# david-zwicker/video-analysis

Hardware: AMD Instinct MI355X
Metric: frames/sec (bg-sub+blur+thresh+CCL) 1080p uint8 (higher is better)
Workload: dtype u8; 1 GPU; cfg3_1080p_full_chain: 1920x1080 uint8, batch 256/GPU, running-mean bg-sub (f64 state) + sigma=5 Gaussian (q8.8) + threshold 20 + 5x5 dilate/erode + 4-connected labelling + object counts; inputs resident in HBM; engine=bg=1 gauss=mfma-i8(ksize=31) thresh=20 morph=2 ccl=4, video=one clip per rank, overlap=off, world_size=1, backend=single process

## Files before the change

### video-analysis_amd/csrc/va_point.hip

```cpp
#include <math.h>

#include "va_common.h"

namespace va {

namespace {

constexpr int kBlock = 256;
constexpr int kVec = 8;

__device__ __forceinline__ uint8_t sat_u8_trunc(double d)
{
    const int v = (int)d;
    return (uint8_t)(v > 255 ? 255 : v);
}

template <int V>
__global__ void __launch_bounds__(kBlock)
bg_mean_u8_kernel(const uint8_t *__restrict__ frames, uint8_t *__restrict__ diff,
                  double *__restrict__ mean, long long n_seen, int n, size_t px)
{
    size_t i0 = ((size_t)blockIdx.x * kBlock + threadIdx.x) * V;
    if (i0 >= px)
        return;
    double m[V];
#pragma unroll
    for (int k = 0; k < V; k++)
        m[k] = mean[i0 + k];
    for (int f = 0; f < n; f++) {
        uint8_t p[V];
        if (V == 8) {
            uint2 v = *reinterpret_cast<const uint2 *>(frames + (size_t)f * px + i0);
            memcpy(p, &v, 8);
        } else {
            p[0] = frames[(size_t)f * px + i0];
        }
        const double dn = (double)(n_seen + f), dn1 = (double)(n_seen + f + 1);
        uint8_t o[V];
#pragma unroll
        for (int k = 0; k < V; k++) {
            double fr = (double)p[k];
            o[k] = sat_u8_trunc(fabs(fr - m[k]));
            m[k] = m[k] * dn / dn1 + fr / dn1;
        }
        if (diff) {
            if (V == 8) {
                uint2 v;
                memcpy(&v, o, 8);
                *reinterpret_cast<uint2 *>(diff + (size_t)f * px + i0) = v;
            } else {
                diff[(size_t)f * px + i0] = o[0];
            }
        }
    }
#pragma unroll
    for (int k = 0; k < V; k++)
        mean[i0 + k] = m[k];
}

__device__ __forceinline__ double div_by_uniform(double x, double d, double y)
{
    const double q = x * y;
    const double r = fma(-q, d, x);
    return fma(r, y, q);
}

__global__ void __launch_bounds__(kBlock)
bg_reciprocals_kernel(double *__restrict__ y, long long n_seen, int n)
{
    const int f = blockIdx.x * kBlock + threadIdx.x;
    if (f < n)
        y[f] = 1.0 / (double)(n_seen + f + 1);
}

struct RecipArgs {
    double r[256];
    double lo[256];
    __device__ double operator[](int f) const { return r[f]; }
};
__device__ __forceinline__ double clear_low9(double y)
{
    return __builtin_bit_cast(double, __builtin_bit_cast(unsigned long long, y) & ~0x1FFull);
}

__device__ __forceinline__ unsigned byte_lane(unsigned w, int k)
{
    return k == 3 ? w >> 24 : (w >> (8 * k)) & 0xFFu;
}
__device__ __forceinline__ unsigned pack_bytes(const int *d)
{
    const unsigned lo = __builtin_amdgcn_perm((unsigned)d[1], (unsigned)d[0], 0x0C0C0400u);
    const unsigned hi = __builtin_amdgcn_perm((unsigned)d[3], (unsigned)d[2], 0x0C0C0400u);
    return __builtin_amdgcn_perm(hi, lo, 0x05040100u);
}

constexpr int kAhead = 8;

template <int V> struct BgGroup {
    typedef unsigned int vec __attribute__((ext_vector_type(V / 4)));
    vec v[kAhead];
    template <bool CLAMP>
    __device__ __forceinline__ void load(const uint8_t *frames, size_t i0, size_t px, int f0, int n)
    {
#pragma unroll
        for (int j = 0; j < kAhead; j++)
            v[j] = __builtin_nontemporal_load(reinterpret_cast<const vec *>(
                frames + (size_t)(CLAMP ? min(f0 + j, n - 1) : f0 + j) * px + i0));
    }
};

template <int V, typename RECIP, bool BOUNDED, bool SPLIT, bool DIFF, bool FULL>
__device__ __forceinline__ void bg_mean_group(const BgGroup<V> &g, double (&m)[V], double &dn, const RECIP &recip,
                                              int f0, int cnt, uint8_t *diff, size_t i0, size_t px)
{
#pragma unroll
    for (int j = 0; j < kAhead; j++) {
        if (!FULL && j >= cnt)
            break;
        const int f = f0 + j;
        const double dn1 = dn + 1.0;
        const double y = recip[f];
        double yh = 0.0, yl = 0.0;
        if constexpr (SPLIT) {
            yh = clear_low9(y);
            yl = recip.lo[f];
        }
        typename BgGroup<V>::vec out;
#pragma unroll
        for (int w = 0; w < V / 4; w++) {
            int d[4];
#pragma unroll
            for (int b = 0; b < 4; b++) {
                const int k = 4 * w + b;
                const double fr = (double)byte_lane(g.v[j][w], b);
                if constexpr (DIFF) {
                    const int a = (int)fabs(fr - m[k]);
                    d[b] = BOUNDED ? a : min(a, 255);
                }
                double q2;
                if constexpr (SPLIT)
                    q2 = fma(fr, yl, fr * yh);
                else
                    q2 = div_by_uniform(fr, dn1, y);
                m[k] = div_by_uniform(m[k] * dn, dn1, y) + q2;
            }
            if constexpr (DIFF)
                out[w] = pack_bytes(d);
        }
        if constexpr (DIFF)
            __builtin_nontemporal_store(out, reinterpret_cast<typename BgGroup<V>::vec *>(diff + (size_t)f * px + i0));
        dn = dn1;
    }
}

template <int V, typename RECIP, bool BOUNDED, bool SPLIT, bool DIFF>
__global__ void __launch_bounds__(kBlock)
bg_mean_u8_fast_kernel(const uint8_t *__restrict__ frames, uint8_t *__restrict__ diff,
                       double *__restrict__ mean, const RECIP recip, double dn0, int n, size_t px)
{
    const size_t i0 = ((size_t)blockIdx.x * kBlock + threadIdx.x) * V;
    if (i0 >= px)
        return;
    double m[V];
#pragma unroll
    for (int k = 0; k < V; k++)
        m[k] = mean[i0 + k];
    double dn = dn0;
    BgGroup<V> a, b;
    a.template load<true>(frames, i0, px, 0, n);
    int f0 = 0;
    for (; f0 + 3 * kAhead <= n; f0 += 2 * kAhead) {
        b.template load<false>(frames, i0, px, f0 + kAhead, n);
        bg_mean_group<V, RECIP, BOUNDED, SPLIT, DIFF, true>(a, m, dn, recip, f0, kAhead, diff, i0, px);
        a.template load<false>(frames, i0, px, f0 + 2 * kAhead, n);
        bg_mean_group<V, RECIP, BOUNDED, SPLIT, DIFF, true>(b, m, dn, recip, f0 + kAhead, kAhead, diff, i0, px);
    }
    for (; f0 < n; f0 += kAhead) {
        const bool more = f0 + kAhead < n;
        if (more)
            b.template load<true>(frames, i0, px, f0 + kAhead, n);
        bg_mean_group<V, RECIP, BOUNDED, SPLIT, DIFF, false>(a, m, dn, recip, f0, min(kAhead, n - f0), diff, i0, px);
        if (more)
            a = b;
    }
#pragma unroll
    for (int k = 0; k < V; k++)
        mean[i0 + k] = m[k];
}

template <int V>
__global__ void __launch_bounds__(kBlock)
bg_static_u8_kernel(const uint8_t *__restrict__ frames, uint8_t *__restrict__ diff,
                    const double *__restrict__ bg, int n, size_t px)
{
    size_t i0 = ((size_t)blockIdx.x * kBlock + threadIdx.x) * V;
    if (i0 >= px)
        return;
    double m[V];
#pragma unroll
    for (int k = 0; k < V; k++)
        m[k] = bg[i0 + k];
    for (int f = 0; f < n; f++) {
        uint8_t p[V], o[V];
        if (V == 8) {
            uint2 v = *reinterpret_cast<const uint2 *>(frames + (size_t)f * px + i0);
            memcpy(p, &v, 8);
        } else {
            p[0] = frames[(size_t)f * px + i0];
        }
#pragma unroll
        for (int k = 0; k < V; k++)
            o[k] = sat_u8_trunc(fabs((double)p[k] - m[k]));
        if (V == 8) {
            uint2 v;
            memcpy(&v, o, 8);
            *reinterpret_cast<uint2 *>(diff + (size_t)f * px + i0) = v;
        } else {
            diff[(size_t)f * px + i0] = o[0];
        }
    }
}

template <int V>
__global__ void __launch_bounds__(kBlock)
bg_ema_u8_kernel(const uint8_t *__restrict__ frames, uint8_t *__restrict__ diff,
                 float *__restrict__ bg, long long n_seen, float rate, int n, size_t px)
{
    size_t i0 = ((size_t)blockIdx.x * kBlock + threadIdx.x) * V;
    if (i0 >= px)
        return;
    float m[V];
#pragma unroll
    for (int k = 0; k < V; k++)
        m[k] = bg[i0 + k];
    for (int f = 0; f < n; f++) {
        uint8_t p[V], o[V];
        if (V == 8) {
            uint2 v = *reinterpret_cast<const uint2 *>(frames + (size_t)f * px + i0);
            memcpy(p, &v, 8);
        } else {
            p[0] = frames[(size_t)f * px + i0];
        }
        const bool first = (n_seen + f) == 0;
#pragma unroll
        for (int k = 0; k < V; k++) {
            float fr = (float)p[k];
            if (first)
                m[k] = fr;
            float d = fr - m[k];
            float a = truncf(fabsf(d));
            o[k] = (uint8_t)(int)(a > 255.0f ? 255.0f : a);
            float step = rate * d;
            m[k] = m[k] + step;
        }
        if (diff) {
            if (V == 8) {
                uint2 v;
                memcpy(&v, o, 8);
                *reinterpret_cast<uint2 *>(diff + (size_t)f * px + i0) = v;
            } else {
                diff[(size_t)f * px + i0] = o[0];
            }
        }
    }
#pragma unroll
    for (int k = 0; k < V; k++)
        bg[i0 + k] = m[k];
}

template <int V>
__global__ void __launch_bounds__(kBlock)
bg_ema_f32_kernel(const float *__restrict__ frames, float *__restrict__ diff,
                  float *__restrict__ bg, long long n_seen, float rate, int n, size_t px)
{
    size_t i0 = ((size_t)blockIdx.x * kBlock + threadIdx.x) * V;
    if (i0 >= px)
        return;
    float m[V];
#pragma unroll
    for (int k = 0; k < V; k++)
        m[k] = bg[i0 + k];
    for (int f = 0; f < n; f++) {
        float p[V], o[V];
        if (V == 4) {
            float4 v = *reinterpret_cast<const float4 *>(frames + (size_t)f * px + i0);
            p[0] = v.x, p[1] = v.y, p[2] = v.z, p[3] = v.w;
        } else {
            p[0] = frames[(size_t)f * px + i0];
        }
        const bool first = (n_seen + f) == 0;
#pragma unroll
        for (int k = 0; k < V; k++) {
            if (first)
                m[k] = p[k];
            float d = p[k] - m[k];
            o[k] = fabsf(d);
            float step = rate * d;
            m[k] = m[k] + step;
        }
        if (diff) {
            if (V == 4)
                *reinterpret_cast<float4 *>(diff + (size_t)f * px + i0) =
                    make_float4(o[0], o[1], o[2], o[3]);
            else
                diff[(size_t)f * px + i0] = o[0];
        }
    }
#pragma unroll
    for (int k = 0; k < V; k++)
        bg[i0 + k] = m[k];
}

template <int V>
__global__ void __launch_bounds__(kBlock)
welford_u8_kernel(const uint8_t *__restrict__ frames, double *__restrict__ mean,
                  double *__restrict__ m2, long long n_seen, int n, size_t px)
{
    size_t i0 = ((size_t)blockIdx.x * kBlock + threadIdx.x) * V;
    if (i0 >= px)
        return;
    double m[V], q[V];
#pragma unroll
    for (int k = 0; k < V; k++) {
        m[k] = mean[i0 + k];
        q[k] = m2[i0 + k];
    }
    for (int f = 0; f < n; f++) {
        uint8_t p[V];
        if (V == 8) {
            uint2 v = *reinterpret_cast<const uint2 *>(frames + (size_t)f * px + i0);
            memcpy(p, &v, 8);
        } else {
            p[0] = frames[(size_t)f * px + i0];
        }
        const double dn1 = (double)(n_seen + f + 1);
#pragma unroll
        for (int k = 0; k < V; k++) {
            double fr = (double)p[k];
            double delta = fr - m[k];
            m[k] = m[k] + delta / dn1;
            q[k] = q[k] + delta * (fr - m[k]);
        }
    }
#pragma unroll
    for (int k = 0; k < V; k++) {
        mean[i0 + k] = m[k];
        m2[i0 + k] = q[k];
    }
}

template <class T>
__device__ __forceinline__ double quotient_as_numpy(T v, double dn1)
{
    return (double)v / dn1;
}
template <>
__device__ __forceinline__ double quotient_as_numpy<float>(float v, double dn1)
{
    return (double)(float)((double)v / (double)(float)dn1);
}

template <class T, bool WELFORD>
__global__ void __launch_bounds__(kBlock)
temporal_stats_kernel(const T *__restrict__ frames, double *__restrict__ mean, double *__restrict__ m2,
                      long long n_seen, int n, size_t px)
{
    const size_t i = (size_t)blockIdx.x * kBlock + threadIdx.x;
    if (i >= px)
        return;
    double m = mean[i], q = WELFORD ? m2[i] : 0.0;
    for (int f = 0; f < n; f++) {
        const T v = frames[(size_t)f * px + i];
        const double dn = (double)(n_seen + f), dn1 = (double)(n_seen + f + 1);
        if (WELFORD) {
            const double fr = (double)v, delta = fr - m;
            m = m + delta / dn1;
            q = q + delta * (fr - m);
        } else {
            m = m * dn / dn1 + quotient_as_numpy<T>(v, dn1);
        }
    }
    mean[i] = m;
    if (WELFORD)
        m2[i] = q;
}

__global__ void __launch_bounds__(kBlock)
threshold_u8_kernel(const uint8_t *__restrict__ src, uint8_t *__restrict__ dst, size_t count,
                    int thresh, int maxval, int vec_ok)
{
    size_t i0 = ((size_t)blockIdx.x * kBlock + threadIdx.x) * 16;
    if (i0 >= count)
        return;
    if (vec_ok && i0 + 16 <= count) {
        uint4 v = *reinterpret_cast<const uint4 *>(src + i0);
        uint8_t p[16];
        memcpy(p, &v, 16);
#pragma unroll
        for (int k = 0; k < 16; k++)
            p[k] = (int)p[k] > thresh ? (uint8_t)maxval : (uint8_t)0;
        memcpy(&v, p, 16);
        *reinterpret_cast<uint4 *>(dst + i0) = v;
    } else {
        for (size_t i = i0; i < count && i < i0 + 16; i++)
            dst[i] = (int)src[i] > thresh ? (uint8_t)maxval : (uint8_t)0;
    }
}

__global__ void __launch_bounds__(kBlock)
time_difference_kernel(const uint8_t *__restrict__ a, const uint8_t *__restrict__ b,
                       int16_t *__restrict__ out, size_t count, int vec_ok)
{
    size_t i0 = ((size_t)blockIdx.x * kBlock + threadIdx.x) * 8;
    if (i0 >= count)
        return;
    if (vec_ok && i0 + 8 <= count) {
        uint2 va_ = *reinterpret_cast<const uint2 *>(a + i0);
        uint2 vb_ = *reinterpret_cast<const uint2 *>(b + i0);
        uint8_t pa[8], pb[8];
        int16_t o[8];
        memcpy(pa, &va_, 8);
        memcpy(pb, &vb_, 8);
#pragma unroll
        for (int k = 0; k < 8; k++)
            o[k] = (int16_t)((int)pa[k] - (int)pb[k]);
        uint4 vo;
        memcpy(&vo, o, 16);
        *reinterpret_cast<uint4 *>(out + i0) = vo;
    } else {
        for (size_t i = i0; i < count && i < i0 + 8; i++)
            out[i] = (int16_t)((int)a[i] - (int)b[i]);
    }
}

__global__ void __launch_bounds__(kBlock)
mono_mean_kernel(const uint8_t *__restrict__ src, uint8_t *__restrict__ dst, size_t pixels)
{
    size_t i = (size_t)blockIdx.x * kBlock + threadIdx.x;
    if (i >= pixels)
        return;
    double s = (double)src[3 * i] + (double)src[3 * i + 1] + (double)src[3 * i + 2];
    dst[i] = (uint8_t)(int)(s / 3.0);
}

__global__ void __launch_bounds__(kBlock)
normalize_u8_kernel(const uint8_t *__restrict__ src, uint8_t *__restrict__ dst, size_t count,
                    double fmin, double fmax, double alpha, double tmin)
{
    size_t i = (size_t)blockIdx.x * kBlock + threadIdx.x;
    if (i >= count)
        return;
    double f = (double)src[i];
    f = f < fmin ? fmin : (f > fmax ? fmax : f);
    double v = (f - fmin) * alpha + tmin;
    int iv = (int)v;
    dst[i] = (uint8_t)iv;
}

}

template <int V, typename RECIP, bool BOUNDED, bool SPLIT>
static void launch_bg_fast(const uint8_t *fr, uint8_t *df, double *mean, const RECIP &recip, double dn0, int n,
                           size_t px, hipStream_t st)
{
    const int grid = cdiv((long long)(px / V), kBlock);
    if constexpr (BOUNDED)
        bg_mean_u8_fast_kernel<V, RECIP, true, SPLIT, true><<<grid, kBlock, 0, st>>>(fr, df, mean, recip, dn0, n, px);
    else if (df)
        bg_mean_u8_fast_kernel<V, RECIP, BOUNDED, SPLIT, true><<<grid, kBlock, 0, st>>>(fr, df, mean, recip, dn0, n, px);
    else
        bg_mean_u8_fast_kernel<V, RECIP, BOUNDED, SPLIT, false><<<grid, kBlock, 0, st>>>(fr, df, mean, recip, dn0, n, px);
}

size_t bg_scratch_bytes(int n) { return sizeof(double) * (size_t)(n > 0 ? n : 1); }

int launch_bg(int mode, int dtype, const void *frames, void *diff, void *state, int64_t n_seen,
              double rate, int n, size_t px, hipStream_t st, double *recip_scratch, bool mean_in_u8_range)
{
    VA_REQUIRE(frames && state, "va_bg_update: frames/state must not be NULL");
    VA_REQUIRE(n >= 0 && px > 0, "va_bg_update: bad sizes n=%d px=%zu", n, px);
    if (n == 0)
        return VA_OK;
    if (dtype == VA_U8) {
        const uint8_t *fr = (const uint8_t *)frames;
        uint8_t *df = (uint8_t *)diff;
        bool vec = (px % kVec == 0) && aligned(fr, 8) && (!df || aligned(df, 8));
        int grid = vec ? cdiv((long long)(px / kVec), kBlock) : cdiv((long long)px, kBlock);
        if (mode == VA_BG_MEAN) {
            const bool wide = px % 16 == 0 && aligned(fr, 16) && (!df || aligned(df, 16));
            const bool countable = n_seen >= -(1ll << 53) && n_seen <= (1ll << 53) - n;
            const bool bounded = mean_in_u8_range && df;
            const double dn0 = (double)n_seen;
            double *mean = (double *)state;
            if (vec && countable && n <= 256) {
                RecipArgs ra;
                for (int f = 0; f < 256; f++) {
                    const double d = (double)(n_seen + (f < n ? f : 0) + 1), y = 1.0 / d;
                    unsigned long long bits;
                    memcpy(&bits, &y, 8);
                    bits &= ~0x1FFull;
                    double yh;
                    memcpy(&yh, &bits, 8);
                    ra.r[f] = y;
                    ra.lo[f] = fma(y, fma(-d, y, 1.0), y - yh);
                }
#ifdef BG_NO_SPLIT
                const bool split = false;
#else
                const bool split = n_seen + n < (1ll << 40);
#endif
                if (wide && bounded && split)
                    launch_bg_fast<16, RecipArgs, true, true>(fr, df, mean, ra, dn0, n, px, st);
                else if (wide && bounded)
                    launch_bg_fast<16, RecipArgs, true, false>(fr, df, mean, ra, dn0, n, px, st);
                else if (wide && split)
                    launch_bg_fast<16, RecipArgs, false, true>(fr, df, mean, ra, dn0, n, px, st);
                else if (wide)
                    launch_bg_fast<16, RecipArgs, false, false>(fr, df, mean, ra, dn0, n, px, st);
                else
                    launch_bg_fast<8, RecipArgs, false, false>(fr, df, mean, ra, dn0, n, px, st);
            } else if (vec && countable && recip_scratch) {
                bg_reciprocals_kernel<<<cdiv(n, kBlock), kBlock, 0, st>>>(recip_scratch, n_seen, n);
                VA_LAUNCH_CHECK("bg_reciprocals_kernel");
                if (wide)
                    launch_bg_fast<16, const double *, false, false>(fr, df, mean, recip_scratch, dn0, n, px, st);
                else
                    launch_bg_fast<8, const double *, false, false>(fr, df, mean, recip_scratch, dn0, n, px, st);
            } else if (vec)
                bg_mean_u8_kernel<8><<<grid, kBlock, 0, st>>>(fr, df, (double *)state, n_seen, n, px);
            else
                bg_mean_u8_kernel<1><<<grid, kBlock, 0, st>>>(fr, df, (double *)state, n_seen, n, px);
        } else if (mode == VA_BG_EMA) {
            if (vec)
                bg_ema_u8_kernel<8><<<grid, kBlock, 0, st>>>(fr, df, (float *)state, n_seen,
                                                            (float)rate, n, px);
            else
                bg_ema_u8_kernel<1><<<grid, kBlock, 0, st>>>(fr, df, (float *)state, n_seen,
                                                            (float)rate, n, px);
        } else if (mode == VA_BG_STATIC) {
            VA_REQUIRE(df, "va_bg_update: static mode needs diff_out");
            if (vec)
                bg_static_u8_kernel<8><<<grid, kBlock, 0, st>>>(fr, df, (const double *)state, n, px);
            else
                bg_static_u8_kernel<1><<<grid, kBlock, 0, st>>>(fr, df, (const double *)state, n, px);
        } else {
            VA_REQUIRE(false, "va_bg_update: unsupported mode %d for u8 frames", mode);
        }
    } else if (dtype == VA_F32) {
        VA_REQUIRE(mode == VA_BG_EMA, "va_bg_update: float32 frames support VA_BG_EMA only");
        const float *fr = (const float *)frames;
        float *df = (float *)diff;
        bool vec = (px % 4 == 0) && aligned(fr, 16) && (!df || aligned(df, 16));
        int grid = vec ? cdiv((long long)(px / 4), kBlock) : cdiv((long long)px, kBlock);
        if (vec)
            bg_ema_f32_kernel<4><<<grid, kBlock, 0, st>>>(fr, df, (float *)state, n_seen,
                                                         (float)rate, n, px);
        else
            bg_ema_f32_kernel<1><<<grid, kBlock, 0, st>>>(fr, df, (float *)state, n_seen,
                                                         (float)rate, n, px);
    } else {
        VA_REQUIRE(false, "va_bg_update: unknown dtype %d", dtype);
    }
    VA_LAUNCH_CHECK("bg kernel");
    return VA_OK;
}

int launch_welford(const uint8_t *frames, double *mean, double *m2, int64_t n_seen, int n,
                   size_t px, hipStream_t st)
{
    VA_REQUIRE(frames && mean && m2, "va_welford_u8: NULL argument");
    if (n <= 0)
        return VA_OK;
    bool vec = (px % kVec == 0) && aligned(frames, 8);
    int grid = vec ? cdiv((long long)(px / kVec), kBlock) : cdiv((long long)px, kBlock);
    if (vec)
        welford_u8_kernel<8><<<grid, kBlock, 0, st>>>(frames, mean, m2, n_seen, n, px);
    else
        welford_u8_kernel<1><<<grid, kBlock, 0, st>>>(frames, mean, m2, n_seen, n, px);
    VA_LAUNCH_CHECK("welford_u8_kernel");
    return VA_OK;
}

int launch_temporal_stats(const void *frames, int dtype, double *mean, double *m2, int64_t n_seen, int n,
                          size_t px, hipStream_t st)
{
    VA_REQUIRE(frames && mean, "temporal statistics: NULL argument");
    VA_REQUIRE(dtype == VA_U8 || dtype == VA_I16 || dtype == VA_F32 || dtype == VA_F64,
               "temporal statistics: frames must be uint8, int16, float32 or float64 (dtype code %d)", dtype);
    if (n <= 0 || px == 0)
        return VA_OK;
    const int grid = cdiv((long long)px, kBlock);
#define VA_TS(T)                                                                                            \
    do {                                                                                                    \
        if (m2)                                                                                             \
            temporal_stats_kernel<T, true><<<grid, kBlock, 0, st>>>((const T *)frames, mean, m2, n_seen, n, px);  \
        else                                                                                                \
            temporal_stats_kernel<T, false><<<grid, kBlock, 0, st>>>((const T *)frames, mean, m2, n_seen, n, px); \
    } while (0)
    if (dtype == VA_U8)
        VA_TS(uint8_t);
    else if (dtype == VA_I16)
        VA_TS(int16_t);
    else if (dtype == VA_F32)
        VA_TS(float);
    else
        VA_TS(double);
#undef VA_TS
    VA_LAUNCH_CHECK("temporal_stats_kernel");
    return VA_OK;
}

int launch_threshold_u8(const uint8_t *src, uint8_t *dst, size_t count, int thresh, int maxval,
                        hipStream_t st)
{
    VA_REQUIRE(src && dst, "va_threshold_u8: NULL argument");
    if (count == 0)
        return VA_OK;
    int vec = aligned(src, 16) && aligned(dst, 16);
    threshold_u8_kernel<<<cdiv((long long)cdiv((long long)count, 16), kBlock), kBlock, 0, st>>>(
        src, dst, count, thresh, maxval, vec);
    VA_LAUNCH_CHECK("threshold_u8_kernel");
    return VA_OK;
}

int launch_time_difference(const uint8_t *a, const uint8_t *b, int16_t *out, size_t count,
                           hipStream_t st)
{
    VA_REQUIRE(a && b && out, "va_time_difference_u8: NULL argument");
    if (count == 0)
        return VA_OK;
    int vec = aligned(a, 8) && aligned(b, 8) && aligned(out, 16);
    time_difference_kernel<<<cdiv((long long)cdiv((long long)count, 8), kBlock), kBlock, 0, st>>>(
        a, b, out, count, vec);
    VA_LAUNCH_CHECK("time_difference_kernel");
    return VA_OK;
}

int launch_mono_mean(const uint8_t *src, uint8_t *dst, size_t pixels, hipStream_t st)
{
    VA_REQUIRE(src && dst, "va_mono_mean_u8: NULL argument");
    if (pixels == 0)
        return VA_OK;
    if (src != dst && launch_pointwise_u8_x4(src, dst, pixels, 3, 3, 0, 0.0, 0.0, 0.0, 0.0, st)) {
        VA_LAUNCH_CHECK("prepare_u8_x4_kernel");
        return VA_OK;
    }
    mono_mean_kernel<<<cdiv((long long)pixels, kBlock), kBlock, 0, st>>>(src, dst, pixels);
    VA_LAUNCH_CHECK("mono_mean_kernel");
    return VA_OK;
}

template <int C, bool SPLIT>
__global__ void __launch_bounds__(kBlock)
channel_planes_kernel(const uint8_t *__restrict__ src, uint8_t *__restrict__ dst, int h, int w, int wp,
                      size_t total_quads)
{
    const size_t t = (size_t)blockIdx.x * kBlock + threadIdx.x;
    if (t >= total_quads)
        return;
    const int qpr = wp / 4;
    const int xq = (int)(t % qpr) * 4;
    const size_t rowi = t / qpr;
    const size_t f = rowi / h, y = rowi % h;
    const uint8_t *inter_c = (SPLIT ? src : nullptr);
    uint8_t *inter = SPLIT ? nullptr : dst;
    const size_t inter_row = rowi * (size_t)w * C;
    const uint8_t *inter_any = SPLIT ? src : dst;
    if (C > 1 && xq + 3 < w && ((w * C) & 3) == 0 && (reinterpret_cast<uintptr_t>(inter_any) & 3) == 0) {
        uint32_t in[C], out[C];
        uint8_t b[4 * C], o[4 * C];
        if (SPLIT) {
#pragma unroll
            for (int c = 0; c < C; c++)
                in[c] = reinterpret_cast<const uint32_t *>(src + inter_row + (size_t)xq * C)[c];
            memcpy(b, in, 4 * C);
#pragma unroll
            for (int c = 0; c < C; c++)
                *reinterpret_cast<uint32_t *>(dst + ((f * C + c) * h + y) * (size_t)wp + xq) =
                    (uint32_t)b[c] | ((uint32_t)b[C + c] << 8) | ((uint32_t)b[2 * C + c] << 16) | ((uint32_t)b[3 * C + c] << 24);
        } else {
#pragma unroll
            for (int c = 0; c < C; c++)
                in[c] = *reinterpret_cast<const uint32_t *>(src + ((f * C + c) * h + y) * (size_t)wp + xq);
            memcpy(b, in, 4 * C);
#pragma unroll
            for (int i = 0; i < 4; i++)
#pragma unroll
                for (int c = 0; c < C; c++)
                    o[i * C + c] = b[4 * c + i];
            memcpy(out, o, 4 * C);
#pragma unroll
            for (int c = 0; c < C; c++)
                reinterpret_cast<uint32_t *>(dst + inter_row + (size_t)xq * C)[c] = out[c];
        }
        return;
    }
    if (SPLIT) {
#pragma unroll
        for (int c = 0; c < C; c++) {
            uint32_t v = 0;
#pragma unroll
            for (int i = 0; i < 4; i++) {
                int x = xq + i;
                x = x < w ? x : 2 * (w - 1) - x;
                x = max(x, 0);
                v |= (uint32_t)inter_c[inter_row + (size_t)x * C + c] << (8 * i);
            }
            *reinterpret_cast<uint32_t *>(dst + ((f * C + c) * h + y) * (size_t)wp + xq) = v;
        }
    } else {
        uint8_t p[C][4];
#pragma unroll
        for (int c = 0; c < C; c++)
            *reinterpret_cast<uint32_t *>(p[c]) =
                *reinterpret_cast<const uint32_t *>(src + ((f * C + c) * h + y) * (size_t)wp + xq);
#pragma unroll
        for (int i = 0; i < 4; i++)
            if (xq + i < w) {
#pragma unroll
                for (int c = 0; c < C; c++)
                    inter[inter_row + (size_t)(xq + i) * C + c] = p[c][i];
            }
    }
}

int launch_channel_planes(const uint8_t *src, uint8_t *dst, int n, int h, int w, int wp, int c,
                          bool split, hipStream_t st)
{
    VA_REQUIRE(src && dst && wp % 4 == 0 && wp >= w && wp - w < w && c >= 1 && c <= 4,
               "channel planes: bad arguments");
    if (n == 0)
        return VA_OK;
    const size_t total = (size_t)n * h * (wp / 4);
    const unsigned grid = (unsigned)((total + kBlock - 1) / kBlock);
#define VA_CP(CC)                                                                                   \
    do {                                                                                            \
        if (split)                                                                                  \
            channel_planes_kernel<CC, true><<<grid, kBlock, 0, st>>>(src, dst, h, w, wp, total);    \
        else                                                                                        \
            channel_planes_kernel<CC, false><<<grid, kBlock, 0, st>>>(src, dst, h, w, wp, total);   \
    } while (0)
    if (c == 1)
        VA_CP(1);
    else if (c == 2)
        VA_CP(2);
    else if (c == 3)
        VA_CP(3);
    else
        VA_CP(4);
#undef VA_CP
    VA_LAUNCH_CHECK("channel_planes_kernel");
    return VA_OK;
}

template <typename E>
__global__ void __launch_bounds__(kBlock)
rot90_kernel(const E *__restrict__ src, E *__restrict__ dst, int h, int w, int k)
{
    __shared__ E tile[32][33];
    const int ho = (k & 1) ? w : h, wo = (k & 1) ? h : w;
    const int tiles_x = (wo + 31) >> 5, tiles_y = (ho + 31) >> 5;
    int t = blockIdx.x;
    const int tx = t % tiles_x;
    t /= tiles_x;
    const int ty = t % tiles_y;
    const size_t f = t / tiles_y;
    const E *in = src + f * (size_t)h * w;
    E *out = dst + f * (size_t)h * w;
    const int lx = threadIdx.x & 31, ly = threadIdx.x >> 5;
    const int i0 = ty * 32, j0 = tx * 32;
#pragma unroll
    for (int r = 0; r < 32; r += 8) {
        const int a = ly + r, b = lx;
        int si, sj;
        if (k == 1) {
            si = j0 + a;
            sj = w - 1 - (i0 + b);
        } else if (k == 2) {
            si = h - 1 - (i0 + a);
            sj = w - 1 - (j0 + b);
        } else if (k == 3) {
            si = h - 1 - (j0 + a);
            sj = i0 + b;
        } else {
            si = i0 + a;
            sj = j0 + b;
        }
        if (si >= 0 && si < h && sj >= 0 && sj < w)
            tile[a][b] = in[(size_t)si * w + sj];
    }
    __syncthreads();
#pragma unroll
    for (int r = 0; r < 32; r += 8) {
        const int i = i0 + ly + r, j = j0 + lx;
        if (i < ho && j < wo) {
            const int di = ly + r, dj = lx;
            E v;
            if (k == 1)
                v = tile[dj][di];
            else if (k == 3)
                v = tile[dj][di];
            else
                v = tile[di][dj];
            out[(size_t)i * wo + j] = v;
        }
    }
}

struct Elem3 { uint8_t b[3]; };
struct Elem6 { uint16_t b[3]; };
struct Elem12 { uint32_t b[3]; };

int launch_rot90(const void *src, void *dst, int n, int h, int w, int elem_bytes, int k,
                 hipStream_t st)
{
    VA_REQUIRE(src && dst && src != dst, "va_rot90: src/dst must be distinct non-NULL");
    VA_REQUIRE(n >= 0 && h > 0 && w > 0, "va_rot90: bad shape (%d,%d,%d)", n, h, w);
    k &= 3;
    if (n == 0)
        return VA_OK;
    const int ho = (k & 1) ? w : h, wo = (k & 1) ? h : w;
    const size_t blocks = (size_t)n * ((ho + 31) / 32) * ((wo + 31) / 32);
    VA_REQUIRE(blocks < ((size_t)1 << 31), "va_rot90: too many tiles");
#define VA_ROT(T) rot90_kernel<T><<<(unsigned)blocks, kBlock, 0, st>>>((const T *)src, (T *)dst, h, w, k)
    switch (elem_bytes) {
    case 1: VA_ROT(uint8_t); break;
    case 2: VA_ROT(uint16_t); break;
    case 3: VA_ROT(Elem3); break;
    case 4: VA_ROT(uint32_t); break;
    case 6: VA_ROT(Elem6); break;
    case 8: VA_ROT(uint64_t); break;
    case 12: VA_ROT(Elem12); break;
    default:
        VA_REQUIRE(false, "va_rot90: unsupported pixel size of %d bytes", elem_bytes);
    }
#undef VA_ROT
    VA_LAUNCH_CHECK("rot90_kernel");
    return VA_OK;
}

int launch_normalize_u8(const uint8_t *src, uint8_t *dst, size_t count, double fmin, double fmax,
                        double alpha, double tmin, hipStream_t st)
{
    VA_REQUIRE(src && dst, "va_normalize_u8: NULL argument");
    if (count == 0)
        return VA_OK;
    if (launch_pointwise_u8_x4(src, dst, count, 1, -1, 1, fmin, fmax, alpha, tmin, st)) {
        VA_LAUNCH_CHECK("prepare_u8_x4_kernel");
        return VA_OK;
    }
    normalize_u8_kernel<<<cdiv((long long)count, kBlock), kBlock, 0, st>>>(src, dst, count, fmin,
                                                                          fmax, alpha, tmin);
    VA_LAUNCH_CHECK("normalize_u8_kernel");
    return VA_OK;
}

}
```

Baseline: 328,900 frames/s.

## Restructure bg-mean prefetch pipeline with explicit waitcnt and prefetched reciprocals

Reworks the double-buffered frame prefetch in the running-mean background kernel so two groups are in flight before compute starts, with explicit s_waitcnt and sched_barrier placement to control when loads are issued and waited on. Reciprocal factors (and split low parts) are now loaded alongside each frame group into registers, with a constant-address-space path for pointer-based reciprocals. The aim is to keep more memory loads outstanding and stop the compiler from serialising loads against compute. In exchange it uses more registers per thread and relies on hand-tuned waitcnt encodings and scheduling barriers, which could hurt occupancy or be fragile.

```diff
diff --git a/video-analysis_amd/csrc/va_point.hip b/video-analysis_amd/csrc/va_point.hip
--- a/video-analysis_amd/csrc/va_point.hip
+++ b/video-analysis_amd/csrc/va_point.hip
@@ -76,7 +76,6 @@
 struct RecipArgs {
     double r[256];
     double lo[256];
-    __device__ double operator[](int f) const { return r[f]; }
 };
 __device__ __forceinline__ double clear_low9(double y)
 {
@@ -96,36 +95,64 @@
 
 constexpr int kAhead = 8;
 
-template <int V> struct BgGroup {
+__device__ __forceinline__ int recip_slot(const RecipArgs &, int f, int) { return f; }
+__device__ __forceinline__ int recip_slot(const double *, int f, int n) { return min(f, n - 1); }
+__device__ __forceinline__ double recip_at(const RecipArgs &r, int slot) { return r.r[slot]; }
+__device__ __forceinline__ double recip_at(const double *r, int slot)
+{
+    return ((const __attribute__((address_space(4))) double *)r)[slot];
+}
+
+template <int V, typename RECIP, bool SPLIT> struct BgGroup {
     typedef unsigned int vec __attribute__((ext_vector_type(V / 4)));
     vec v[kAhead];
+    double y[kAhead], lo[kAhead];
     template <bool CLAMP>
-    __device__ __forceinline__ void load(const uint8_t *frames, size_t i0, size_t px, int f0, int n)
+    __device__ __forceinline__ void load(const uint8_t *frames, const RECIP &recip, size_t i0, size_t px, int f0,
+                                         int n)
     {
-#pragma unroll
-        for (int j = 0; j < kAhead; j++)
+        __builtin_amdgcn_s_waitcnt(0xC07F);
+#pragma unroll
+        for (int j = 0; j < kAhead; j++) {
             v[j] = __builtin_nontemporal_load(reinterpret_cast<const vec *>(
                 frames + (size_t)(CLAMP ? min(f0 + j, n - 1) : f0 + j) * px + i0));
+            __builtin_amdgcn_sched_barrier(0);
+        }
+#pragma unroll
+        for (int j = 0; j < kAhead; j++) {
+            const int slot = CLAMP ? recip_slot(recip, f0 + j, n) : f0 + j;
+            y[j] = recip_at(recip, slot);
+            if constexpr (SPLIT)
+                lo[j] = recip.lo[slot];
+        }
+        __builtin_amdgcn_sched_barrier(0);
+    }
+    __device__ __forceinline__ void arrived()
+    {
+#pragma unroll
+        for (int j = 0; j < kAhead; j++)
+            asm volatile("" : "+v"(v[j]));
     }
 };
 
 template <int V, typename RECIP, bool BOUNDED, bool SPLIT, bool DIFF, bool FULL>
-__device__ __forceinline__ void bg_mean_group(const BgGroup<V> &g, double (&m)[V], double &dn, const RECIP &recip,
-                                              int f0, int cnt, uint8_t *diff, size_t i0, size_t px)
-{
+__device__ __forceinline__ void bg_mean_group(const BgGroup<V, RECIP, SPLIT> &g, double (&m)[V], double &dn, int f0,
+                                              int cnt, uint8_t *diff, size_t i0, size_t px)
+{
+    typedef typename BgGroup<V, RECIP, SPLIT>::vec vec;
 #pragma unroll
     for (int j = 0; j < kAhead; j++) {
         if (!FULL && j >= cnt)
             break;
         const int f = f0 + j;
         const double dn1 = dn + 1.0;
-        const double y = recip[f];
+        const double y = g.y[j];
         double yh = 0.0, yl = 0.0;
         if constexpr (SPLIT) {
             yh = clear_low9(y);
-            yl = recip.lo[f];
-        }
-        typename BgGroup<V>::vec out;
+            yl = g.lo[j];
+        }
+        vec out;
 #pragma unroll
         for (int w = 0; w < V / 4; w++) {
             int d[4];
@@ -148,7 +175,7 @@
                 out[w] = pack_bytes(d);
         }
         if constexpr (DIFF)
-            __builtin_nontemporal_store(out, reinterpret_cast<typename BgGroup<V>::vec *>(diff + (size_t)f * px + i0));
+            __builtin_nontemporal_store(out, reinterpret_cast<vec *>(diff + (size_t)f * px + i0));
         dn = dn1;
     }
 }
@@ -166,23 +193,33 @@
     for (int k = 0; k < V; k++)
         m[k] = mean[i0 + k];
     double dn = dn0;
-    BgGroup<V> a, b;
-    a.template load<true>(frames, i0, px, 0, n);
+    BgGroup<V, RECIP, SPLIT> a, b;
     int f0 = 0;
-    for (; f0 + 3 * kAhead <= n; f0 += 2 * kAhead) {
-        b.template load<false>(frames, i0, px, f0 + kAhead, n);
-        bg_mean_group<V, RECIP, BOUNDED, SPLIT, DIFF, true>(a, m, dn, recip, f0, kAhead, diff, i0, px);
-        a.template load<false>(frames, i0, px, f0 + 2 * kAhead, n);
-        bg_mean_group<V, RECIP, BOUNDED, SPLIT, DIFF, true>(b, m, dn, recip, f0 + kAhead, kAhead, diff, i0, px);
-    }
-    for (; f0 < n; f0 += kAhead) {
-        const bool more = f0 + kAhead < n;
-        if (more)
-            b.template load<true>(frames, i0, px, f0 + kAhead, n);
-        bg_mean_group<V, RECIP, BOUNDED, SPLIT, DIFF, false>(a, m, dn, recip, f0, min(kAhead, n - f0), diff, i0, px);
-        if (more)
-            a = b;
-    }
+    if (n >= 3 * kAhead) {
+        a.template load<false>(frames, recip, i0, px, 0, n);
+        b.template load<false>(frames, recip, i0, px, kAhead, n);
+        bg_mean_group<V, RECIP, BOUNDED, SPLIT, DIFF, true>(a, m, dn, 0, kAhead, diff, i0, px);
+        for (f0 = kAhead; f0 + 3 * kAhead <= n; f0 += 2 * kAhead) {
+            a.template load<false>(frames, recip, i0, px, f0 + kAhead, n);
+            bg_mean_group<V, RECIP, BOUNDED, SPLIT, DIFF, true>(b, m, dn, f0, kAhead, diff, i0, px);
+            b.template load<false>(frames, recip, i0, px, f0 + 2 * kAhead, n);
+            bg_mean_group<V, RECIP, BOUNDED, SPLIT, DIFF, true>(a, m, dn, f0 + kAhead, kAhead, diff, i0, px);
+        }
+        b.arrived();
+    } else {
+        b.template load<true>(frames, recip, i0, px, 0, n);
+#pragma unroll
+        for (int k = 0; k < V; k++)
+            asm volatile("" : "+v"(m[k]));
+        b.arrived();
+    }
+    for (; f0 + kAhead < n; f0 += kAhead) {
+        a.template load<true>(frames, recip, i0, px, f0 + kAhead, n);
+        bg_mean_group<V, RECIP, BOUNDED, SPLIT, DIFF, true>(b, m, dn, f0, kAhead, diff, i0, px);
+        a.arrived();
+        b = a;
+    }
+    bg_mean_group<V, RECIP, BOUNDED, SPLIT, DIFF, false>(b, m, dn, f0, n - f0, diff, i0, px);
 #pragma unroll
     for (int k = 0; k < V; k++)
         mean[i0 + k] = m[k];
```

Measured after the change: 332,900 frames/s (median of 6 runs). 1.01x the previous value.
